# ErickRosete/tacorl

Hardware: AMD Instinct MI355X
Metric: offline grad-steps/sec (batch=256, 84x84 RGB) (higher is better)
Workload: dtype bf16; 1 GPU; tacorl actor-critic training_step, frozen LMP (BASELINE configs[1]); per_gpu_batch=256, global_batch=256, window=16, image=84x84x3, frames=fp32 CHW (reference batch schema), latent_plan=16, n_action_samples=4, phase=Q (epoch>=bc_epochs), action_decoder_loss=every step (reference behaviour), parallelism=dp1, hip_graph=True, losses_finite=True

## Files before the change

### include/tacorl_hip.h

```cpp
#ifndef TACORL_HIP_H
#define TACORL_HIP_H
#include <stddef.h>
#ifdef __cplusplus
extern "C" {
#endif

typedef void* tacorl_stream_t;

#define TACORL_MAXP 16
enum { TACORL_F32 = 0, TACORL_BF16 = 1 };
enum { TACORL_ACT_NONE = 0, TACORL_ACT_RELU = 1, TACORL_ACT_SILU = 2, TACORL_ACT_TANH = 3 };

int tacorl_hip_version(void);
int tacorl_hip_init(int device);
const char* tacorl_hip_last_error(void);
int tacorl_time_mark(unsigned long long* marks, int slot, tacorl_stream_t stream);
int tacorl_time_spin(unsigned long long* marks, int slot, long ticks, tacorl_stream_t stream);

int tacorl_linear_fwd(int nprob, const float* const* x, int ldx, const float* const* w,
                      const float* const* b, float* const* y, float* const* z, const int* M,
                      int K, int N, int act, int compute_dtype, tacorl_stream_t stream);
size_t tacorl_linear_add_fwd_ws_bytes(int nprob, const int* M, int K, int N);
int tacorl_linear_add_fwd(int nprob, const float* const* x, int ldx, const float* const* w,
                          const float* const* b, const float* const* addend, int ld_add, float* const* y,
// ... 161 lines not shown
                               void* ws, size_t ws_bytes, tacorl_stream_t stream);

int tacorl_pack_images(const float* src, long img_pitch, int src_nchw, void* dst, int dst_dtype,
                       int n, int C, int H, int W, tacorl_stream_t stream);
int tacorl_pack_images_batch(int njobs, const float* const* src, const long* img_pitch, void* const* dst,
                             const int* n_img, int dst_dtype, int H, int W, tacorl_stream_t stream);
int tacorl_pack_images_window_batch(int njobs, const float* const* src, const long* img_pitch, void* const* dst,
                                    const int* n_img, void* const* dst_first, void* const* dst_last,
                                    const int* window, int dst_dtype, int H, int W, tacorl_stream_t stream);
int tacorl_pack_images_u8_batch(int njobs, const void* const* src, const long* img_pitch_bytes, void* const* dst,
                                const int* n_img, int dst_dtype, int H, int W, tacorl_stream_t stream);
int tacorl_pack_images_u8_gather_batch(int njobs, const void* const* src, const long* img_pitch_bytes,
                                       const long* const* index, const int* index_stride, void* const* dst,
                                       const int* n_img, int dst_dtype, int H, int W, tacorl_stream_t stream);
int tacorl_gather_frames_u8(const void* frames, long frame_bytes, const long* index, void* dst, long n,
                            tacorl_stream_t stream);
int tacorl_pack_images_u8_aug_batch(int njobs, const void* const* src, const long* img_pitch_bytes,
                                    void* const* dst, const int* const* shift, const float* const* jitter,
                                    const int* n_img, int dst_dtype, int H, int W, int pad,
                                    tacorl_stream_t stream);
int tacorl_pack_images_u8_resize_aug_gather_batch(int njobs, const void* const* src, const long* img_pitch_bytes,
                                                  const long* const* index, const int* index_stride, void* const* dst,
                                                  const int* const* shift, const float* const* jitter, const int* n_img,
                                                  int dst_dtype, int src_H, int src_W, int H, int W, int pad,
                                                  tacorl_stream_t stream);
int tacorl_resize_frames_u8(const void* src, long src_pitch_bytes, void* dst, long dst_pitch_bytes, long n, int src_H,
                            int src_W, int H, int W, tacorl_stream_t stream);
int tacorl_pack_images_u8_aug_gather_batch(int njobs, const void* const* src, const long* img_pitch_bytes,
                                           const long* const* index, const int* index_stride, void* const* dst,
                                           const int* const* shift, const float* const* jitter, const int* n_img,
                                           int dst_dtype, int H, int W, int pad, tacorl_stream_t stream);
int tacorl_stage_transition(const void* disp, int disp_dtype, float* reward, float* done, int B,
                            const float* acts_src, float* acts_dst, long n_acts, tacorl_stream_t stream);
int tacorl_sample_transitions(const long* possible_steps, long n_possible, const long* ep_start, const long* ep_end,
                              int n_episodes, const long* nn_ptr, long n_nn, const long* nn_val, const float* actions,
                              const long* idx, const long* strategy, const long* disp, const double* u_choice,
                              long current_horizon, long n_frames, int B, int A, long* ids, float* action,
                              float* reward, float* done, int* status, tacorl_stream_t stream);
int tacorl_sample_relay(const long* episode_lookup, long n_items, const long* ep_start, const long* ep_end, int n_episodes,
                        const float* actions, long n_frames, const long* idx, const double* u_low, const double* u_high,
                        long max_low_level_window, long max_high_level_window, int B, int A, long* ids, float* action,
                        int* status, tacorl_stream_t stream);
int tacorl_sample_d4rl_windows(const long* episode_lookup, long n_items, const long* ep_start, const long* ep_end,
                               int n_episodes, const float* observations, const float* actions, long n_frames,
                               const long* idx, const long* window, const long* disp, int B, int Tmax, int S, int A,
                               int G, int min_window, float threshold, float* obs, float* act, float* goal,
                               float* reached, float* done, long* window_size, long* ids, int* status,
                               tacorl_stream_t stream);
int tacorl_sample_play_windows(const long* episode_lookup, long n_items, const long* ep_start, const long* ep_end,
                               int n_episodes, const long* nn_ptr, long n_nn, const long* nn_val, const float* actions,
                               long n_frames, long last_end, const long* idx, const long* window, const long* strategy,
                               const long* disp, const long* noise_step, const double* u_choice,
                               const double* u_random_state, int B, int Tmax, int A, int min_window, long* ids, float* act,
                               long* disp_out, long* window_size, int* status, tacorl_stream_t stream);
int tacorl_copy_cols(const float* src, int ld_src, float* dst, int ld_dst, int rows, int cols,
                     int src_row_mod, int accumulate, tacorl_stream_t stream);
int tacorl_copy_cols_batch(int n, const float* const* src, const int* ld_src, float* const* dst,
                           const int* ld_dst, const int* rows, const int* cols,
                           const int* src_row_mod, const int* accumulate, tacorl_stream_t stream);
int tacorl_vec_rows_max_blocks(void);
int tacorl_vec_rows(const float* obs, const float* goal, const float* acts_main, const float* act_pi,
                    const float* act_next, float* const* out, void* const* out_bf16, int B, int T, int S, int G, int A,
                    int n, int lds, int ldq, tacorl_stream_t stream);
int tacorl_reduce_rows_mod(const float* in, int ld_in, float* out, int ld_out, int B, int cols,
                           int reps, tacorl_stream_t stream);
int tacorl_reduce_rows_mod_batch(int n, const float* const* in, int ld_in, float* const* out, int ld_out, int B,
// ... 199 lines not shown
```

### tacorl_amd/_lib.py

```python
import ctypes as C
import os

HERE = os.path.dirname(os.path.abspath(__file__))
LIB_PATH = os.environ.get("TACORL_HIP_LIB") or os.path.join(HERE, "lib", "libtacorl_hip.so")

F32, BF16 = 0, 1
ACT_NONE, ACT_RELU, ACT_SILU, ACT_TANH = 0, 1, 2, 3
MAXP = 16

LOG_SLOTS = [
    "alpha_loss", "alpha", "actor_loss", "bellman_q1_loss", "bellman_q2_loss", "conservative_q1_loss",
    "conservative_q2_loss", "q1_loss", "q2_loss", "alpha_prime", "alpha_prime_loss", "q1_data", "q1_random",
    "q1_policy", "q2_data", "q2_random", "q2_policy", "action_loss",
]

_p, _i, _l, _f, _sz = C.c_void_p, C.c_int, C.c_long, C.c_float, C.c_size_t
_SIGS = {
    "tacorl_hip_version": (_i, []),
    "tacorl_hip_init": (_i, [_i]),
    "tacorl_hip_last_error": (C.c_char_p, []),
    "tacorl_time_mark": (_i, [_p, _i, _p]),
    "tacorl_time_spin": (_i, [_p, _i, _l, _p]),
    "tacorl_linear_fwd": (_i, [_i, _p, _i, _p, _p, _p, _p, _p, _i, _i, _i, _i, _p]),
    "tacorl_linear_add_fwd_ws_bytes": (_sz, [_i, _p, _i, _i]),
# ... 83 lines not shown
    "tacorl_encoder_fused_wpk_bytes": (_l, []),
    "tacorl_encoder_fused_supported": (_i, [_i, _i]),
    "tacorl_encoder_fused_act_format": (_i, [_i, _i]),
    "tacorl_encoder_pack_weights": (_i, [_i, _p, _p, _p]),
    "tacorl_encoder_fwd_fused": (_i, [_i, _p, _p, _p, _p, _p, _p, _i, _i, _p]),
    "tacorl_encoder_fwd_fused_wg": (_i, [_i, _p, _p, _p, _p, _p, _p, _i, _i, _i, _p]),
    "tacorl_encoder_src_entry_bytes": (_l, []),
    "tacorl_encoder_src_supported": (_i, [_p, _l, _l, _l, _i, _i]),
    "tacorl_encoder_src_fill": (_i, [_p, _i, _p, _p, _p, _p, _i, _i, _p]),
    "tacorl_encoder_fwd_fused_src": (_i, [_i, _p, _p, _p, _p, _p, _p, _p, _i, _i, _i, _p]),
    "tacorl_encoder_bwd_fused_ws_bytes": (_sz, [_i, _p, _i, _i]),
    "tacorl_encoder_bwd_fused": (_i, [_i, _p, _p, _p, _p, _p, _p, _i, _i, _i, _p, _sz, _p]),
    "tacorl_encoder_bwd_fused_pack": (_i, [_i, _p, _p, _i, _i, _p, _sz, _p]),
    "tacorl_encoder_bwd_fused_head": (_i, [_i, _p, _p, _p, _p, _i, _i, _i, _p, _sz, _p]),
    "tacorl_encoder_bwd_fused_fc_wgrad": (_i, [_i, _p, _p, _p, _p, _i, _i, _i, _p, _sz, _p]),
    "tacorl_encoder_bwd_fused_conv": (_i, [_i, _p, _p, _p, _p, _p, _i, _i, _i, _i, _p, _sz, _p]),
    "tacorl_encoder_bwd_fused_conv_parts": (_i, [_i, _p, _p, _p, _p, _p, _i, _i, _i, _i, _i, _p, _sz, _p]),
    "tacorl_mlp_param_layout": (_l, [_i, _p, _p, _p]),
    "tacorl_mlp_act_layout": (_l, [_i, _i, _p, _p, _p, _p]),
    "tacorl_mlp_fwd": (_i, [_i, _p, _i, _p, _p, _p, _i, _p, _p, _i, _p]),
    "tacorl_mlp_bwd_ws_bytes": (_sz, [_i, _p, _i, _p]),
    "tacorl_mlp_bwd": (_i, [_i, _p, _i, _p, _p, _p, _i, _p, _p, _i, _p, _i, _p, _p, _i, _i, _p, _sz, _p]),
    "tacorl_pack_images": (_i, [_p, _l, _i, _p, _i, _i, _i, _i, _i, _p]),
    "tacorl_pack_images_batch": (_i, [_i, _p, _p, _p, _p, _i, _i, _i, _p]),
    "tacorl_pack_images_window_batch": (_i, [_i, _p, _p, _p, _p, _p, _p, _p, _i, _i, _i, _p]),
    "tacorl_pack_images_u8_batch": (_i, [_i, _p, _p, _p, _p, _i, _i, _i, _p]),
    "tacorl_pack_images_u8_gather_batch": (_i, [_i, _p, _p, _p, _p, _p, _p, _i, _i, _i, _p]),
    "tacorl_pack_images_u8_aug_gather_batch": (_i, [_i, _p, _p, _p, _p, _p, _p, _p, _p, _i, _i, _i, _i, _p]),
    "tacorl_pack_images_u8_resize_aug_gather_batch": (_i, [_i, _p, _p, _p, _p, _p, _p, _p, _p, _i, _i, _i, _i, _i, _i, _p]),
    "tacorl_gather_frames_u8": (_i, [_p, _l, _p, _p, _l, _p]),
    "tacorl_resize_frames_u8": (_i, [_p, _l, _p, _l, _l, _i, _i, _i, _i, _p]),
    "tacorl_pack_images_u8_aug_batch": (_i, [_i, _p, _p, _p, _p, _p, _p, _i, _i, _i, _i, _p]),
    "tacorl_stage_transition": (_i, [_p, _i, _p, _p, _i, _p, _p, _l, _p]),
    "tacorl_sample_transitions": (_i, [_p, _l, _p, _p, _i, _p, _l, _p, _p, _p, _p, _p, _p, _l, _l, _i, _i, _p, _p, _p, _p, _p, _p]),
    "tacorl_sample_relay": (_i, [_p, _l, _p, _p, _i, _p, _l, _p, _p, _p, _l, _l, _i, _i, _p, _p, _p, _p]),
    "tacorl_sample_d4rl_windows": (_i, [_p, _l, _p, _p, _i, _p, _p, _l, _p, _p, _p, _i, _i, _i, _i, _i, _i, _f, _p, _p, _p, _p, _p, _p,
                                        _p, _p, _p]),
    "tacorl_sample_play_windows": (_i, [_p, _l, _p, _p, _i, _p, _l, _p, _p, _l, _l, _p, _p, _p, _p, _p, _p, _p, _i, _i, _i, _i,
                                        _p, _p, _p, _p, _p, _p]),
    "tacorl_copy_cols": (_i, [_p, _i, _p, _i, _i, _i, _i, _i, _p]),
    "tacorl_copy_cols_batch": (_i, [_i, _p, _p, _p, _p, _p, _p, _p, _p, _p]),
    "tacorl_vec_rows_max_blocks": (_i, []),
    "tacorl_vec_rows": (_i, [_p, _p, _p, _p, _p, _p, _p, _i, _i, _i, _i, _i, _i, _i, _i, _p]),
    "tacorl_reduce_rows_mod": (_i, [_p, _i, _p, _i, _i, _i, _i, _p]),
    "tacorl_reduce_rows_mod_batch": (_i, [_i, _p, _i, _p, _i, _i, _i, _i, _p]),
    "tacorl_uniform_actions": (_i, [_p, _p, _i, _i, _i, _i, _p]),
    "tacorl_tanh_normal_sample": (_i, [_p, _i, _p, _p, _i, _p, _i, _p, _p, _i, _i, _i, _p]),
    "tacorl_tanh_normal_sample_batch": (_i, [_i, _p, _i, _p, _p, _p, _p, _i, _p, _p, _p, _i, _i, _p, _p, _i, _i, _i, _p]),
    "tacorl_alpha_loss": (_i, [_p, _i, _p, _f, _f, _p, _p, _p]),
    "tacorl_alpha_loss_step": (_i, [_p, _i, _p, _f, _p, _p, _p, _p, _f, _p, _p]),
    "tacorl_actor_qmin": (_i, [_p, _p, _p, _i, _p, _p, _p, _f, _p, _p]),
    "tacorl_actor_head_bwd": (_i, [_p, _i, _p, _p, _p, _p, _i, _p, _i, _p, _p, _f, _p, _i, _i, _i, _p, _p]),
    "tacorl_tanh_normal_nll": (_i, [_p, _i, _p, _i, _i, _i, _i, _f, _p, _p, _p]),
    "tacorl_cql_ws_bytes": (_sz, [_i]),
    "tacorl_cql_loss": (_i, [_p] * 13 + [_i, _i, _i, _f, _f, _f, _f, _f, _i, _f, _p, _p, _p, _sz, _p]),
    "tacorl_adam_ws_bytes": (_sz, [_l]),
    "tacorl_adam_step": (_i, [_p, _p, _p, _p, _l, _f, _f, _p, _p, _f, _p, _sz, _p]),
    "tacorl_adam_batch_ws_bytes": (_sz, [_i]),
    "tacorl_adam_step_batch": (_i, [_i, _p, _p, _p, _p, _p, _p, _p, _p, _p, _p, _p, _sz, _p]),
    "tacorl_adam_step_batch_mirror": (_i, [_i, _p, _p, _p, _p, _p, _p, _p, _p, _p, _p, _p, _p, _p, _sz, _p]),
    "tacorl_cem_supported": (_i, [_i, _i, _i, _i, _i, _i]),
    "tacorl_cem_ws_bytes": (_sz, [_i, _i, _i, _i, _i, _i, _i]),
    "tacorl_cem_refine": (_i, [_i, _i, _p, _p, _p, _p, _p, _p, _i, _i, _i, _i, _i, _i, _i, _f, _f, _f, _i, _i, _p, _p, _p, _p, _p,
                               _p, _sz, _p]),
    "tacorl_knn_l2_supported": (_i, [_i, _i]),
    "tacorl_knn_l2_tile": (_i, []),
# ... 94 lines not shown
```

### tacorl_amd/csrc/rl_ops.hip

```cpp
#include <stdio.h>

#include "../../include/tacorl_hip.h"
#include "common.h"

#define LAUNCH_OK() (hipGetLastError() == hipSuccess ? TACORL_OK : TACORL_ELAUNCH)

__device__ __forceinline__ float softplusf(float x) {
  return x > 20.f ? x : log1pf(expf(x));
}
__device__ __forceinline__ float block_sum_256(float v, float* sh) {
  v = wave_sum(v);
  __syncthreads();
  if ((threadIdx.x & 63) == 0) sh[threadIdx.x >> 6] = v;
  __syncthreads();
  return sh[0] + sh[1] + sh[2] + sh[3];
}

template <typename OutT>
__global__ void pack_images_kernel(const float* __restrict__ src, long img_pitch, int src_nchw,
                                   OutT* __restrict__ dst, int n, int C, int HW) {
  const long total = (long)n * HW;
  for (long i = (long)blockIdx.x * blockDim.x + threadIdx.x; i < total; i += (long)gridDim.x * blockDim.x) {
    const long img = i / HW;
    const int px = (int)(i - img * HW);
    const float* s = src + img * img_pitch;
    OutT* d = dst + i * C;
    for (int c = 0; c < C; c++) d[c] = (OutT)(src_nchw ? s[(long)c * HW + px] : s[(long)px * C + c]);
  }
}
extern "C" int tacorl_pack_images(const float* src, long img_pitch, int src_nchw, void* dst, int dst_dtype,
                                  int n, int C, int H, int W, tacorl_stream_t stream) {
  if (n <= 0) return TACORL_OK;
  const long total = (long)n * H * W;
  const int blocks = (int)((total + 255) / 256 > 4096 ? 4096 : (total + 255) / 256);
  if (dst_dtype == TACORL_BF16)
    hipLaunchKernelGGL(pack_images_kernel<__bf16>, dim3(blocks), dim3(256), 0, (hipStream_t)stream, src, img_pitch,
// ... 149 lines not shown
  }
  if (m == 0) return TACORL_OK;
  const int blocks = (int)((mx + 255) / 256 > 8192 ? 8192 : (mx + 255) / 256);
  if (dst_dtype == TACORL_BF16)
    hipLaunchKernelGGL(pack_u8_batch_kernel<__bf16>, dim3(blocks, m), dim3(256), 0, (hipStream_t)stream, t, (int)(bytes / 16));
  else
    hipLaunchKernelGGL(pack_u8_batch_kernel<float>, dim3(blocks, m), dim3(256), 0, (hipStream_t)stream, t, (int)(bytes / 16));
  return LAUNCH_OK();
}

__global__ void stage_transition_kernel(const void* __restrict__ disp, int disp_dtype, float* __restrict__ reward,
                                        float* __restrict__ done, int B, const float* __restrict__ acts_src,
                                        float* __restrict__ acts_dst, long n_acts) {
  const long i = (long)blockIdx.x * blockDim.x + threadIdx.x;
  if (i < B) {
    bool one;
    if (disp_dtype == 0) one = static_cast<const float*>(disp)[i] == 1.0f;
    else if (disp_dtype == 1) one = static_cast<const long long*>(disp)[i] == 1;
    else if (disp_dtype == 2) one = static_cast<const int*>(disp)[i] == 1;
    else one = static_cast<const unsigned char*>(disp)[i] == 1;
    const float r = one ? 1.0f : 0.0f;
    reward[i] = r;
    if (done) done[i] = r;
  }
  for (long k = i; k < n_acts; k += (long)gridDim.x * blockDim.x) acts_dst[k] = acts_src[k];
}
extern "C" int tacorl_stage_transition(const void* disp, int disp_dtype, float* reward, float* done, int B,
                                       const float* acts_src, float* acts_dst, long n_acts, tacorl_stream_t stream) {
  if (!disp || !reward || B < 1 || disp_dtype < 0 || disp_dtype > 3 || (n_acts > 0 && (!acts_src || !acts_dst))) return TACORL_EINVAL;
  const long work = n_acts > B ? n_acts : B;
  const int blocks = (int)((work + 255) / 256 > 1024 ? 1024 : (work + 255) / 256);
  hipLaunchKernelGGL(stage_transition_kernel, dim3(blocks < (B + 255) / 256 ? (B + 255) / 256 : blocks), dim3(256), 0,
                     (hipStream_t)stream, disp, disp_dtype, reward, done, B, acts_src, acts_dst, n_acts);
  return LAUNCH_OK();
}

__global__ void copy_cols_kernel(const float* __restrict__ src, int ld_src, float* __restrict__ dst, int ld_dst,
                                 int rows, int cols, int src_row_mod, int accumulate) {
  const long total = (long)rows * cols;
  for (long i = (long)blockIdx.x * blockDim.x + threadIdx.x; i < total; i += (long)gridDim.x * blockDim.x) {
    const int r = (int)(i / cols), c = (int)(i - (long)r * cols);
    const int rs = src_row_mod > 0 ? r % src_row_mod : r;
    const float v = src[(long)rs * ld_src + c];
    float* d = dst + (long)r * ld_dst + c;
    *d = accumulate ? *d + v : v;
  }
}
extern "C" int tacorl_copy_cols(const float* src, int ld_src, float* dst, int ld_dst, int rows, int cols,
                                int src_row_mod, int accumulate, tacorl_stream_t stream) {
  if (rows <= 0 || cols <= 0) return TACORL_OK;
  const long total = (long)rows * cols;
  const int blocks = (int)((total + 255) / 256 > 2048 ? 2048 : (total + 255) / 256);
  hipLaunchKernelGGL(copy_cols_kernel, dim3(blocks), dim3(256), 0, (hipStream_t)stream, src, ld_src, dst, ld_dst, rows,
                     cols, src_row_mod, accumulate);
  return LAUNCH_OK();
}

#define COPY_MAXB 32
struct CopyTbl {
  const float* src[COPY_MAXB];
  float* dst[COPY_MAXB];
  int ld_src[COPY_MAXB], ld_dst[COPY_MAXB], rows[COPY_MAXB], cols[COPY_MAXB], mod[COPY_MAXB], acc[COPY_MAXB];
};
__global__ void copy_cols_batch_kernel(CopyTbl t) {
  const int d = blockIdx.y, cols = t.cols[d], mod = t.mod[d], acc = t.acc[d];
  const long total = (long)t.rows[d] * cols;
// ... 858 lines not shown
```

### tacorl_amd/encoder_stage.py

```python
import torch

from . import ops
from ._lib import BF16, F32, call

EF_MAXP = 16
EBW_MAXP = 8


def image_flag(img_dtype):
    return BF16 if img_dtype == torch.bfloat16 else F32


def fused_fwd_ok(hw, compute, img_dtype):
    return compute == BF16 and img_dtype == torch.bfloat16 and bool(ops.L.lib().tacorl_encoder_fused_supported(*hw))


def fused_bwd_ok(hw, compute, img_dtype, n_imgs):
    return fused_fwd_ok(hw, compute, img_dtype) and ops.L.lib().tacorl_encoder_bwd_fused_ws_bytes(
        len(n_imgs), ops.int_array(n_imgs), *hw) > 0


def fused_saves(hw, compute, img_dtype, n_imgs):
    return fused_bwd_ok(hw, compute, img_dtype, n_imgs) or (
        fused_fwd_ok(hw, compute, img_dtype) and ops.L.lib().tacorl_encoder_fused_act_format(*hw) == 2)
# ... 38 lines not shown
    for c in cams:
        groups.setdefault((tuple(hw[c]), bool(ok(c))), []).append(c)
    for (_, good), cs in groups.items():
        out += [cs] if good and sum(n_problems(c) for c in cs) <= limit else [[c] for c in cs]
    return out


def problem_src(x):
    return x[7] if len(x) > 7 else None


class SourceTable:

    def __init__(self, device, n):
        self.esz = int(ops.L.lib().tacorl_encoder_src_entry_bytes())
        self.n, self.buf = n, torch.zeros(n * self.esz, dtype=torch.uint8, device=device)

    def entry(self, i):
        return self.buf.data_ptr() + i * self.esz

    @staticmethod
    def ok(base, img_pitch, hw):
        H, W = hw
        return bool(ops.L.lib().tacorl_encoder_src_supported(ops.C.c_void_p(base), img_pitch, H * W, W, H, W))

    def fill(self, sources, hw):
        H, W = hw
        n, Lg = len(sources), ops.C.c_long * len(sources)
        assert 0 < n <= self.n
        call("tacorl_encoder_src_fill", ops.ptr(self.buf), n, ops.ptr_array([b for b, _ in sources]), Lg(*[p for _, p in sources]),
             Lg(*[H * W] * n), Lg(*[W] * n), H, W, ops.stream())


def launch_fused(pr, packs, hw, max_wg=0):
    srcs = [problem_src(x) for x in pr]
    if any(srcs):
        assert not any(s_ and x[5] for s_, x in zip(srcs, pr)), "a problem with a backward reads the packed image"
        call("tacorl_encoder_fwd_fused_src", len(pr), ops.ptr_array([x[0] for x in pr]), ops.ptr_array(srcs),
             ops.ptr_array([packs.buffer(x[1], x[6]) for x in pr]), ops.ptr_array([x[1].enc(x[6]) for x in pr]),
             ops.ptr_array([x[2] for x in pr]), ops.ptr_array([x[3] if x[5] else None for x in pr]),
             ops.int_array([x[4] for x in pr]), *hw, int(max_wg), ops.stream())
        return
    call("tacorl_encoder_fwd_fused_wg", len(pr), ops.ptr_array([x[0] for x in pr]),
         ops.ptr_array([packs.buffer(x[1], x[6]) for x in pr]), ops.ptr_array([x[1].enc(x[6]) for x in pr]),
         ops.ptr_array([x[2] for x in pr]), ops.ptr_array([x[3] if x[5] else None for x in pr]),
         ops.int_array([x[4] for x in pr]), *hw, int(max_wg), ops.stream())


def encode(groups, problems, hw, compute, img_dtype, packs, fused, saves, launch, pack_per_camera=True, per_layer_last=False):
    def per_layer(pr):
        for c in dict.fromkeys(x[6] for x in pr):
            prc = [x for x in pr if x[6] == c]
            call("tacorl_encoder_fwd", len(prc), ops.ptr_array([x[0] for x in prc]), ops.ptr_array([x[1].enc(c) for x in prc]),
                 ops.ptr_array([x[2] for x in prc]), ops.ptr_array([x[3] for x in prc]), ops.int_array([x[4] for x in prc]),
                 *hw[c], image_flag(img_dtype), compute, ops.stream())

    slow = []
    for cs in groups:
        pr = [x for c in cs for x in problems(c)]
        if fused(cs[0]):
            unsaved = lambda x: x[5] and not saves(x[6])
            slow += [x for x in pr if unsaved(x)]
            pr = [x for x in pr if not unsaved(x)]
            pairs = list(dict.fromkeys((x[1], x[6]) for c in cs for x in pr if x[6] == c))
            for part in ([[p for p in pairs if p[1] == c] for c in cs] if pack_per_camera else [pairs]):
                packs.pack_stale(part)
# ... 8 lines not shown
```

### tacorl_amd/modules/tacorl/tacorl.py

```python
import torch

from ... import encoder_stage as stage
from ... import image_ingest as ingest
from ... import ops
from ..._lib import call, ptr
from ...encoder_stage import image_flag
from ..common import register_views
from ..cql.cql_offline_lightning import CQL_Offline
from .latent_plan import LatentPlanShell


class TACORL(LatentPlanShell, CQL_Offline):
    def __init__(self, *args, **kwargs):
        self.action_loss_every_n_steps = kwargs.pop("action_loss_every_n_steps", 1)
        super().__init__(*args, **kwargs)

    def build_networks(self):
        from ..play_lmp.play_lmp_for_rl import PlayLMP, load_play_lmp

        lmp = self.__dict__.pop("_play_lmp", None)
        if lmp is None:
            lmp = load_play_lmp(self.play_lmp_dir, self.lmp_epoch_to_load, self.overwrite_lmp_cfg, device=self.dev,
                                compute_dtype=self.compute, image_dtype=self.img_dtype, unsafe_pickle=self.lmp_unsafe_pickle)
        assert isinstance(lmp, PlayLMP)
# ... 18 lines not shown
            init_views_(q.views)
            n = q.head_off - q.genc_off
            q.param[q.genc_off: q.genc_off + n].copy_(lmp.net.param[lmp.net.genc_off: lmp.net.genc_off + n])
        self.sync_targets()
        self._register()
        self.lmp_net, self.pr, self.ad = lmp.net, lmp.pr, lmp.ad
        enc_views = {k[len("encoder."):]: v for k, v in lmp.net.views.items() if k.startswith("encoder.")}
        register_views(self, "perceptual_encoder.", enc_views, requires_grad=False)
        register_views(self, "plan_recognition.", lmp.pr.blk.views, requires_grad=False)
        if self.ad is not None:
            self._adopt_decoder()
        self._T = None
        from ..inference import attach_rollout_surface

        attach_rollout_surface(self, e.actor, cams, goal_cams, self.action_dim, False, lmp_net=self.lmp_net,
                               lmp_cams=self.action_decoder_modalities, ad=self.ad)

    def _ensure_seq(self, B, T, hw):
        if self._T == (B, T, tuple(sorted(hw.items()))):
            return
        ops.note_alloc()
        dev = self.dev
        self.frames = ingest.LazyImages({c: torch.zeros(B * T, *hw[c], 3, device=dev, dtype=self.img_dtype) for c in self.all_modalities})
        self.f_out = {c: torch.zeros(B * T, 32, device=dev) for c in self.all_modalities}
        self.f_act = {c: torch.zeros(ops.encoder_act_layout(B * T, *hw[c])[1], device=dev) for c in self.all_modalities}
        npr = len(self.plan_recognition_modalities)
        self.pr_in = torch.zeros(B * T, 32 * npr, device=dev)
        e = self.engine
        assert e.action.shape == (B, self.action_dim) and e.action.dtype == torch.float32
        self.plan, self.reward = e.action, e.reward
        self.engine.extra_enc = [dict(cam=c, img=self.frames.raw(c), net=self.lmp_net, out=self.f_out[c],
                                      act=self.f_act[c], n=B * T) for c in self.all_modalities]
        self.src_tbl = {c: stage.SourceTable(dev, 2) for c in sorted(set(self.all_modalities) | set(self.engine.cams))}
        self._folded = None
        self._T = (B, T, tuple(sorted(hw.items())))

    def _stage_small(self, batch, noise, B, T):
        e = self.engine
        disp, acts = batch["disp"], batch["actions"] if self.ad is not None else None
        dd = {torch.float32: 0, torch.int64: 1, torch.int32: 2, torch.uint8: 3, torch.bool: 3}.get(disp.dtype)
        if (dd is not None and disp.is_cuda and disp.is_contiguous() and disp.numel() == B
                and (acts is None or (acts.is_cuda and acts.is_contiguous() and acts.dtype == torch.float32
                                      and acts.shape == self.acts.shape))):
            call("tacorl_stage_transition", ptr(disp), dd, ptr(self.reward), ptr(e.done), B,
                 ptr(acts) if acts is not None else None, ptr(self.acts) if acts is not None else None,
                 acts.numel() if acts is not None else 0, ops.stream())
        else:
            if acts is not None:
                self.acts.copy_(acts)
            self.reward.copy_(disp == 1)
            e.done.copy_(self.reward)
        e.set_noise(noise)

    def _fold_ok(self, f, c, T, batch):
        e, hw = self.engine, f.hw[c]
        if not (f.form == "f32_nchw" and f.aug is None and T >= 2 and e.use_fused and stage.fused_fwd_ok(hw, self.compute, self.img_dtype)):
            return False
        goal = batch["goal"][c] if c in e.cams else None
        if c in e.cams and not (c in e.slot and list(e.slot[c]) == ["obs", "goal", "next"] and goal.is_cuda and goal.is_contiguous()
                                and goal.dtype == torch.float32 and ingest.vector_ok(
                [ingest.PackJob(goal.data_ptr(), 3 * hw[0] * hw[1], 0, 1)], f.form, hw)):
            return False
        v, simg = f.frames[c], 3 * hw[0] * hw[1]
        return stage.SourceTable.ok(v.data_ptr(), simg, hw) and stage.SourceTable.ok(v.data_ptr() + 4 * (T - 1) * simg, T * simg, hw)

    def _stage_frames(self, batch, noise, nchw=True, fold=False):
        from ...data.replay import wait_ready

        wait_ready(batch)
        f = ingest.window_form(batch, nchw)
        B, T, hw, aug = f.B, f.T, f.hw, f.aug
        self.engine.extra_normal = {"eps_pr": (B, self.action_dim)}
        self.engine.ensure_batch(B, {c: hw[c] for c in self.engine.cams})
        self.eps_pr = self.engine.extra_noise["eps_pr"]
        self._ensure_seq(B, T, hw)
        e = self.engine
        if self.ad is not None and (getattr(self, "acts", None) is None or self.acts.shape[:2] != (B, T)):
            ops.note_alloc()
            self.acts = torch.zeros(B, T, 7, device=self.dev)
        if getattr(self, "_stage_stream", None) is None:
            self._stage_stream = torch.cuda.Stream(device=self.dev)
        main = torch.cuda.current_stream()
        side = self._stage_stream if getattr(self, "stage_side", True) else main
        side.wait_stream(main)
        with torch.cuda.stream(side):
            self._stage_small(batch, noise, B, T)
        u8, Job, ip = f.form in ingest.U8_FORMS, ingest.PackJob, None if f.ids is None else f.ids.data_ptr()
        cams_all = sorted(set(self.all_modalities) | set(e.cams))
        for c in cams_all:
            v = f.frames[c]
            assert v.is_cuda and v.is_contiguous() and v.dtype == (torch.uint8 if u8 else torch.float32)
        folded = tuple(c for c in cams_all if fold and self._fold_ok(f, c, T, batch))
        if folded != self._folded:
            ops.note_alloc()
            self._folded = folded
        self.frames.drop()
        e.X3.drop()
        e.fp_src = {c: {"next": self.src_tbl[c].entry(1)} for c in folded if c in e.cams}
        for x in e.extra_enc:
            x["src"] = self.src_tbl[x["cam"]].entry(0) if x["cam"] in folded else None
        for c in cams_all:
            v = f.frames[c]
            src, simg = v.data_ptr(), 3 * f.src_hw[c][0] * f.src_hw[c][1]
            if c in folded:
                self.src_tbl[c].fill([(src, simg), (src + 4 * (T - 1) * simg, T * simg)], hw[c])
                form, shw = f.form, f.src_hw[c]
                later = lambda jobs, c=c, keep=v, form=form, shw=shw: ingest.pack(jobs, form, self.img_dtype, shw, hw[c])
                if c in self.all_modalities:
                    self.frames.defer(c, lambda c=c, later=later, src=src, simg=simg: later([Job(src, simg, self.frames.raw(c).data_ptr(), B * T)]))
                if c in e.cams:
                    x3, slot = e.X3.raw(c).data_ptr(), B * 3 * hw[c][0] * hw[c][1] * e.X3.raw(c).element_size()
                    ingest.pack([Job(src, T * simg, x3, B), Job(batch["goal"][c].data_ptr(), simg, x3 + slot, B)], form, self.img_dtype, shw, hw[c])
                    e.X3.defer(c, lambda later=later, src=src, simg=simg, x3=x3, slot=slot: later([Job(src + 4 * (T - 1) * simg, T * simg, x3 + 2 * slot, B)]))
                continue
            jobs, roles = [], []
            if c in self.all_modalities:
                jobs, roles = [Job(src, simg, self.frames.raw(c).data_ptr(), B * T, ip, 1)], ["window"]
            if c in e.cams:
                x3, slot = e.X3.raw(c).data_ptr(), B * 3 * hw[c][0] * hw[c][1] * e.X3.raw(c).element_size()
                if ip is not None:
                    jobs += [Job(src, simg, x3, B, ip, T), Job(src, simg, x3 + slot, B, ip + 8 * B * T, 1),
                             Job(src, simg, x3 + 2 * slot, B, ip + 8 * (T - 1), T)]
                else:
                    g = batch["goal"][c]
                    assert g.is_cuda and g.is_contiguous() and g.dtype == v.dtype
                    jobs += [Job(src, T * simg, x3, B), Job(g.data_ptr(), simg, x3 + slot, B),
                             Job(src + v.element_size() * (T - 1) * simg, T * simg, x3 + 2 * slot, B)]
                roles += ["obs", "goal", "next"]
            if aug is not None:
                jobs = [j._replace(**ingest.window_tables(aug, c, r, T)) for j, r in zip(jobs, roles)]
            if len(jobs) == 4 and T >= 2 and ingest.vector_ok(jobs, f.form, hw[c]):
                ingest.pack_window(jobs, T, self.img_dtype, hw[c])
            else:
                ingest.pack(jobs, f.form, self.img_dtype, f.src_hw[c], hw[c], aug["pad"][c] if aug is not None else None)
        main.wait_stream(side)
        return B, T, hw

    def _ad_due(self):
        k = self.action_loss_every_n_steps
        return self.ad is not None and (self.finetune_action_decoder or k <= 1 or (self._step_count + 1) % k == 0)

    def _device_front(self, B, T, hw, optimize, with_ad=True):
        e = self.engine
        ops.mark("front:start")
        if getattr(self, "_pr_stream", None) is None:
            self._pr_stream, self._side_stream = torch.cuda.Stream(device=self.dev), torch.cuda.Stream(device=self.dev)
        main = torch.cuda.current_stream()
        mods = self.plan_recognition_modalities
        emb, ld = (self.f_out[mods[0]], 32) if len(mods) == 1 else (self.pr_in, self.pr_in.shape[1])
        ad_prep, ad_prepared = None, False
        if (with_ad and optimize and self.finetune_action_decoder and getattr(self, "ad_early_prepare", True)
                and self.ad._bwd_fast(B, self.compute)):
            self._side_stream.wait_stream(main)
            with torch.cuda.stream(self._side_stream):
                self.ad.refresh_mirrors(B, T - 1)
                ad_prepared = self.ad.prepare_backward(B, T - 1, self.compute)
                ad_prep = torch.cuda.Event()
                ad_prep.record(self._side_stream)
        split = with_ad and (T >= 24 or (optimize and self.finetune_action_decoder))
        forked = []

        def fork_branches():
            forked.append(self._fork_pr_ad(B, T, main, mods, emb, ld, with_ad, optimize, ad_prep, ad_prepared))

        if not (split and e.encode_split(fork_branches)):
            e._encode_all()
        ops.mark("front:encoded")
        if not forked:
            fork_branches()
        ready, ad_on_side = forked[0]
        e.action_ready = ready
        e.phase_a(encoded=True, optimize=optimize)
        if ad_prep is not None:
            main.wait_stream(self._side_stream)
        segmented = self._segmented() or not self._use_graph
        if with_ad and not ad_on_side:
            if segmented:
# ... 28 lines not shown
            ready = torch.cuda.Event()
            ready.record(self._pr_stream)
            if with_ad and not ad_on_side:
                if ad_prep is not None:
                    self._pr_stream.wait_event(ad_prep)
                self.ad.loss_step(self, self.acts, self.plan, B, T, True, defer_update=self._defer_ad_update(),
                                  mirrors_current=ad_prep is not None, prepared=ad_prepared)
        if ad_on_side:
            self._side_stream.wait_event(ready)
            with torch.cuda.stream(self._side_stream):
                ops.mark("ad:start")
                self.ad.loss_step(self, self.acts, self.plan, B, T, False, frozen=not self.finetune_action_decoder,
                                  rows_current=rows_current)
                ops.mark("ad:end")
            self._ad_join = self._side_stream
        return ready, ad_on_side

    def get_pr_latent_plan(self, batch, noise=None, nchw=True):
        B, T, hw = self._stage_frames(batch, noise, nchw)
        xd = image_flag(self.img_dtype)
        for c in self.all_modalities:
            H, W = hw[c]
            call("tacorl_encoder_fwd", 1, ops.ptr_array([self.frames[c]]), ops.ptr_array([self.lmp_net.enc(c)]),
                 ops.ptr_array([self.f_out[c]]), ops.ptr_array([self.f_act[c]]), ops.int_array([B * T]), H, W, xd,
                 self.compute, ops.stream())
        for j, c in enumerate(self.plan_recognition_modalities):
            ops.copy_cols(self.f_out[c], 0, 32, self.pr_in, 32 * j, self.pr_in.shape[1], B * T, 32)
        head = self.pr.forward(self.pr_in, self.pr_in.shape[1], B, T, self.compute, inference=True)
        call("tacorl_pr_sample", ptr(head), ptr(self.eps_pr), ptr(self.plan), None, None, B, self.action_dim,
             float(self.pr.min_std), ops.stream())
        return self.plan

    def _step(self, batch, noise, optimize, log_type, nchw=True):
        B, T, hw = self._stage_frames(batch, noise, nchw, fold=getattr(self, "fp32_ingest", True))
        with_ad = self._ad_due()
        key = ("tacorl", B, T, tuple(sorted(hw.items())), self.current_epoch < self.bc_epochs, optimize, with_ad)
        e, bc = self.engine, self.current_epoch < self.bc_epochs
        ad_update = with_ad and optimize and self.finetune_action_decoder and self._defer_ad_update()

        def tail():
            e.phase_c(optimize)
            self._join_ad()
            if ad_update:
                self.ad.update(self)
            ops.mark("step:end")

        segmented = self._segmented()
        ad_ft = optimize and self.finetune_action_decoder
        ad_side = with_ad and segmented and self._use_graph
        side = None
        if ad_side and ad_ft:
            side = (0, lambda: self.ad.loss_step(self, self.acts, self.plan, B, T, True, defer_update=True), 1)
        elif ad_side:
            side = (0, lambda: self.ad.loss_step(self, self.acts, self.plan, B, T, False, frozen=not self.finetune_action_decoder))
        def allreduce_grads():
            if ad_update:
                self._join_ad()
            e.allreduce_grads()

        self._run_segments(key, [lambda: self._device_front(B, T, hw, optimize, with_ad and not ad_side),
                                 lambda: e.phase_b(bc, optimize), tail],
                           [e.allreduce_alpha, allreduce_grads], side=side)
        self._publish_logs(log_type, extra=("action_loss",) if with_ad else ())
```

Before: 1314 grad-steps/s.

## Merge step-front staging into one table-driven kernel launched inside the graph

Replaces the separate per-step front kernels (transition staging, reward/done/action copy, goal and current-frame packing, per-camera source-table fills) with a single device table filled once per step and one step_front kernel launched at the start of the device front. The aim is to cut launch count and the gaps between small kernels and side-stream syncs before the encoder runs. In exchange it adds a fill kernel plus host-side table assembly. It also moves staging onto the main stream, which gives up the earlier overlap on the side stream. It only applies when the configuration is non-segmented and all cameras share one folded resolution.

```diff
diff --git a/include/tacorl_hip.h b/include/tacorl_hip.h
--- a/include/tacorl_hip.h
+++ b/include/tacorl_hip.h
@@ -217,6 +217,22 @@
                                            int dst_dtype, int H, int W, int pad, tacorl_stream_t stream);
 int tacorl_stage_transition(const void* disp, int disp_dtype, float* reward, float* done, int B,
                             const float* acts_src, float* acts_dst, long n_acts, tacorl_stream_t stream);
+#define TACORL_SF_MAXCAM 4
+#define TACORL_SF_MAXJOBS 8
+#define TACORL_SF_NOFFSETS 15
+long tacorl_step_front_table_bytes(void);
+int tacorl_step_front_offsets(long* offsets);
+int tacorl_step_front_supported(int nsrc, const float* const* src_base, const long* src_pitch, int njobs,
+                                const float* const* pack_src, const long* pack_pitch, void* const* pack_dst,
+                                const int* pack_n, const void* disp, int disp_dtype, const float* reward, int B,
+                                const float* acts_src, const float* acts_dst, long n_acts, int H, int W);
+int tacorl_step_front_assemble(void* host_table, int nsrc, const float* const* src_base, const long* src_pitch, int njobs,
+                               const float* const* pack_src, const long* pack_pitch, void* const* pack_dst,
+                               const int* pack_n, const void* disp, int disp_dtype, float* reward, float* done, int B,
+                               const float* acts_src, float* acts_dst, long n_acts, int H, int W);
+int tacorl_step_front_fill(void* table, const void* host_table, tacorl_stream_t stream);
+int tacorl_step_front(const void* table, int njobs, int max_images, int B, long n_acts, int H, int W,
+                      tacorl_stream_t stream);
 int tacorl_sample_transitions(const long* possible_steps, long n_possible, const long* ep_start, const long* ep_end,
                               int n_episodes, const long* nn_ptr, long n_nn, const long* nn_val, const float* actions,
                               const long* idx, const long* strategy, const long* disp, const double* u_choice,
diff --git a/scratch/front_launches.py b/scratch/front_launches.py
--- /dev/null
+++ b/scratch/front_launches.py
@@ -0,0 +1,25 @@
+import csv, glob, sys, collections
+f = glob.glob(sys.argv[1] + "/**/*kernel_trace.csv", recursive=True)[0]
+rows = sorted(csv.DictReader(open(f)), key=lambda r: int(r["Start_Timestamp"]))
+name = lambda r: r["Kernel_Name"].replace("(anonymous namespace)::", "").replace("void ", "")
+enc = [i for i, r in enumerate(rows) if name(r).startswith("encoder_fused_kernel")]
+FRONT = ("pack_nchw3", "stage_transition", "ef_src_fill", "step_front", "distribution", "normal", "uniform")
+for k in (150, 180):
+    a = enc[k]
+    i = a - 1
+    while i > 0 and any(s in name(rows[i]) for s in FRONT):
+        i -= 1
+    t0 = int(rows[i]["End_Timestamp"])
+    print(f"-- step {k}: us since the previous replay's last kernel ended (start, duration, queue, kernel)")
+    for r in rows[i - 1:a + 2]:
+        d = (int(r["End_Timestamp"]) - int(r["Start_Timestamp"])) / 1e3
+        print(f"{(int(r['Start_Timestamp']) - t0) / 1e3:9.1f} us  {d:7.1f}  q{r.get('Queue_Id', '?')}  {name(r)[:100]}")
+tot, cnt = collections.Counter(), collections.Counter()
+for r in rows:
+    n = name(r)
+    if any(s in n for s in FRONT) or n.startswith("encoder_fused_kernel"):
+        tot[n[:80]] += (int(r["End_Timestamp"]) - int(r["Start_Timestamp"])) / 1e3
+        cnt[n[:80]] += 1
+print("-- mean us per dispatch (dispatches)")
+for n in tot:
+    print(f"{tot[n] / cnt[n]:8.1f}  ({cnt[n]})  {n}")
diff --git a/scratch/front_marks.py b/scratch/front_marks.py
--- /dev/null
+++ b/scratch/front_marks.py
@@ -0,0 +1,31 @@
+import os, sys, json
+sys.path.insert(0, os.path.join(os.path.dirname(os.path.abspath(__file__)), ".."))
+import torch, bench
+from tacorl_amd import _lib, ops
+dev = torch.device("cuda:0"); _lib.call("tacorl_hip_init", 0)
+res = {}
+for traced in (False, True):
+    reader = ops.trace_marks(dev) if traced else None
+    mod = bench.build_module(dev, "bf16", 16, 1)
+    batch = bench.synth_batch(256, 16, 84, 84, dev, 1)
+    mod.enable_graph(); mod.log_every_n_steps = 50
+    def run(n):
+        for i in range(n): mod.training_step(batch, i)
+    run(20); torch.cuda.synchronize()
+    per, spans, fronts = [], [], []
+    for burst in range(6):
+        e0, e1 = torch.cuda.Event(enable_timing=True), torch.cuda.Event(enable_timing=True)
+        e0.record(); run(200); e1.record(); torch.cuda.synchronize()
+        ms = e0.elapsed_time(e1) / 200
+        per.append(ms)
+        if traced:
+            m = dict(reader())
+            span = m["step:end"] - m["front:start"]
+            spans.append(span); fronts.append(ms * 1000 - span)
+    key = "traced" if traced else "untraced"
+    res[key + "_ms_per_step"] = [round(x, 4) for x in per]
+    if traced:
+        res["span_us"] = [round(x, 1) for x in spans]
+        res["front_us"] = [round(x, 1) for x in fronts]
+        res["last_marks"] = [(n, round(t, 1)) for n, t in reader()]
+print("FRONT " + json.dumps(res), flush=True)
diff --git a/tacorl_amd/_lib.py b/tacorl_amd/_lib.py
--- a/tacorl_amd/_lib.py
+++ b/tacorl_amd/_lib.py
@@ -139,6 +139,12 @@
     "tacorl_resize_frames_u8": (_i, [_p, _l, _p, _l, _l, _i, _i, _i, _i, _p]),
     "tacorl_pack_images_u8_aug_batch": (_i, [_i, _p, _p, _p, _p, _p, _p, _i, _i, _i, _i, _p]),
     "tacorl_stage_transition": (_i, [_p, _i, _p, _p, _i, _p, _p, _l, _p]),
+    "tacorl_step_front_table_bytes": (_l, []),
+    "tacorl_step_front_offsets": (_i, [_p]),
+    "tacorl_step_front_supported": (_i, [_i, _p, _p, _i, _p, _p, _p, _p, _p, _i, _p, _i, _p, _p, _l, _i, _i]),
+    "tacorl_step_front_assemble": (_i, [_p, _i, _p, _p, _i, _p, _p, _p, _p, _p, _i, _p, _p, _i, _p, _p, _l, _i, _i]),
+    "tacorl_step_front_fill": (_i, [_p, _p, _p]),
+    "tacorl_step_front": (_i, [_p, _i, _i, _i, _l, _i, _i, _p]),
     "tacorl_sample_transitions": (_i, [_p, _l, _p, _p, _i, _p, _l, _p, _p, _p, _p, _p, _p, _l, _l, _i, _i, _p, _p, _p, _p, _p, _p]),
     "tacorl_sample_relay": (_i, [_p, _l, _p, _p, _i, _p, _l, _p, _p, _p, _l, _l, _i, _i, _p, _p, _p, _p]),
     "tacorl_sample_d4rl_windows": (_i, [_p, _l, _p, _p, _i, _p, _p, _l, _p, _p, _p, _i, _i, _i, _i, _i, _i, _f, _p, _p, _p, _p, _p, _p,
diff --git a/tacorl_amd/csrc/rl_ops.hip b/tacorl_amd/csrc/rl_ops.hip
--- a/tacorl_amd/csrc/rl_ops.hip
+++ b/tacorl_amd/csrc/rl_ops.hip
@@ -1,7 +1,11 @@
+#include <stddef.h>
 #include <stdio.h>
+#include <string.h>
 
 #include "../../include/tacorl_hip.h"
 #include "common.h"
+#include "encoder_fused.h"
+#include "step_front_table.h"
 
 #define LAUNCH_OK() (hipGetLastError() == hipSuccess ? TACORL_OK : TACORL_ELAUNCH)
 
@@ -217,6 +221,114 @@
   const int blocks = (int)((work + 255) / 256 > 1024 ? 1024 : (work + 255) / 256);
   hipLaunchKernelGGL(stage_transition_kernel, dim3(blocks < (B + 255) / 256 ? (B + 255) / 256 : blocks), dim3(256), 0,
                      (hipStream_t)stream, disp, disp_dtype, reward, done, B, acts_src, acts_dst, n_acts);
+  return LAUNCH_OK();
+}
+
+static_assert(sizeof(SFSrc) == sizeof(EFSrc) && offsetof(SFSrc, base) == offsetof(EFSrc, base) &&
+                  offsetof(SFSrc, img_pitch) == offsetof(EFSrc, img_pitch) && offsetof(SFSrc, plane_pitch) == offsetof(EFSrc, plane_pitch) &&
+                  offsetof(SFSrc, row_pitch) == offsetof(EFSrc, row_pitch),
+              "the front table's source entries are the fused encoder's");
+__global__ void step_front_fill_kernel(SFTable* __restrict__ tbl, SFTable f) {
+  const long* s = reinterpret_cast<const long*>(&f);
+  long* d = reinterpret_cast<long*>(tbl);
+  for (int i = threadIdx.x; i < (int)(sizeof(SFTable) / 8); i += blockDim.x) d[i] = s[i];
+}
+__global__ void step_front_kernel(const SFTable* __restrict__ t) {
+  const int j = blockIdx.y;
+  if (j < t->njobs) {
+    const int HW = t->HW, q4 = HW / 4;
+    const long total = (long)t->pack_n[j] * q4, pitch = t->pack_pitch[j];
+    const float* __restrict__ src = t->pack_src[j];
+    __bf16* __restrict__ dst = reinterpret_cast<__bf16*>(t->pack_dst[j]);
+    for (long q = (long)blockIdx.x * blockDim.x + threadIdx.x; q < total; q += (long)gridDim.x * blockDim.x) {
+      const long img = q / q4;
+      const int p = (int)(q - img * q4) * 4;
+      const float* s = src + img * pitch + p;
+      const f32x4 r = *reinterpret_cast<const f32x4*>(s), g = *reinterpret_cast<const f32x4*>(s + HW),
+                  b = *reinterpret_cast<const f32x4*>(s + 2 * HW);
+      const float v[12] = {r[0], g[0], b[0], r[1], g[1], b[1], r[2], g[2], b[2], r[3], g[3], b[3]};
+      __bf16* d = dst + (img * HW + p) * 3;
+#pragma unroll
+      for (int k = 0; k < 3; k++)
+        *reinterpret_cast<bf16x4*>(d + 4 * k) = bf16x4{(__bf16)v[4 * k], (__bf16)v[4 * k + 1], (__bf16)v[4 * k + 2], (__bf16)v[4 * k + 3]};
+    }
+    return;
+  }
+  if (j != (int)gridDim.y - 1) return;
+  const long i = (long)blockIdx.x * blockDim.x + threadIdx.x;
+  const int B = t->B, disp_dtype = t->disp_dtype;
+  const void* __restrict__ disp = t->disp;
+  if (i < B) {
+    bool one;
+    if (disp_dtype == 0) one = static_cast<const float*>(disp)[i] == 1.0f;
+    else if (disp_dtype == 1) one = static_cast<const long long*>(disp)[i] == 1;
+    else if (disp_dtype == 2) one = static_cast<const int*>(disp)[i] == 1;
+    else one = static_cast<const unsigned char*>(disp)[i] == 1;
+    const float r = one ? 1.0f : 0.0f;
+    t->reward[i] = r;
+    if (t->done) t->done[i] = r;
+  }
+  const long n_acts = t->n_acts;
+  const float* __restrict__ acts_src = t->acts_src;
+  float* __restrict__ acts_dst = t->acts_dst;
+  for (long k = i; k < n_acts; k += (long)gridDim.x * blockDim.x) acts_dst[k] = acts_src[k];
+}
+extern "C" long tacorl_step_front_table_bytes(void) { return (long)sizeof(SFTable); }
+extern "C" int tacorl_step_front_offsets(long* out) {
+  if (!out) return TACORL_EINVAL;
+  const long o[TACORL_SF_NOFFSETS] = {
+      (long)offsetof(SFTable, src),      (long)offsetof(SFTable, pack_src),   (long)offsetof(SFTable, pack_dst),
+      (long)offsetof(SFTable, pack_pitch), (long)offsetof(SFTable, pack_n),   (long)offsetof(SFTable, disp),
+      (long)offsetof(SFTable, reward),   (long)offsetof(SFTable, done),       (long)offsetof(SFTable, acts_src),
+      (long)offsetof(SFTable, acts_dst), (long)offsetof(SFTable, n_acts),     (long)offsetof(SFTable, disp_dtype),
+      (long)offsetof(SFTable, B),        (long)offsetof(SFTable, njobs),      (long)offsetof(SFTable, HW)};
+  for (int i = 0; i < TACORL_SF_NOFFSETS; i++) out[i] = o[i];
+  return TACORL_OK;
+}
+extern "C" int tacorl_step_front_supported(int nsrc, const float* const* src_base, const long* src_pitch, int njobs,
+                                           const float* const* pack_src, const long* pack_pitch, void* const* pack_dst,
+                                           const int* pack_n, const void* disp, int disp_dtype, const float* reward, int B,
+                                           const float* acts_src, const float* acts_dst, long n_acts, int H, int W) {
+  if (!sf_supported(nsrc, src_base, src_pitch, njobs, pack_src, pack_pitch, pack_dst, pack_n, disp, disp_dtype, reward, B, acts_src,
+                    acts_dst, n_acts, H, W))
+    return 0;
+  for (int i = 0; i < nsrc; i++)
+    if (!tacorl_encoder_src_supported(src_base[i], src_pitch[i], (long)H * W, W, H, W)) return 0;
+  return 1;
+}
+extern "C" int tacorl_step_front_assemble(void* host_table, int nsrc, const float* const* src_base, const long* src_pitch,
+                                          int njobs, const float* const* pack_src, const long* pack_pitch,
+                                          void* const* pack_dst, const int* pack_n, const void* disp, int disp_dtype,
+                                          float* reward, float* done, int B, const float* acts_src, float* acts_dst,
+                                          long n_acts, int H, int W) {
+  if (!host_table || !tacorl_step_front_supported(nsrc, src_base, src_pitch, njobs, pack_src, pack_pitch, pack_dst, pack_n, disp,
+                                                  disp_dtype, reward, B, acts_src, acts_dst, n_acts, H, W))
+    return TACORL_EINVAL;
+  sf_assemble(static_cast<SFTable*>(host_table), nsrc, src_base, src_pitch, njobs, pack_src, pack_pitch, pack_dst, pack_n, disp,
+              disp_dtype, reward, done, B, acts_src, acts_dst, n_acts, H, W);
+  return TACORL_OK;
+}
+extern "C" int tacorl_step_front_fill(void* table, const void* host_table, tacorl_stream_t stream) {
+  if (!table || !host_table || ((uintptr_t)table & 7)) return TACORL_EINVAL;
+  SFTable f;
+  memcpy(&f, host_table, sizeof(SFTable));
+  if (!sf_table_sane(f)) return TACORL_EINVAL;
+  hipLaunchKernelGGL(step_front_fill_kernel, dim3(1), dim3(64), 0, (hipStream_t)stream, static_cast<SFTable*>(table), f);
+  return LAUNCH_OK();
+}
+extern "C" int tacorl_step_front(const void* table, int njobs, int max_images, int B, long n_acts, int H, int W,
+                                 tacorl_stream_t stream) {
+  if (!table || njobs < 0 || njobs > TACORL_SF_MAXJOBS || (njobs > 0 && max_images < 1) || B < 1 || n_acts < 0 || H < 1 || W < 1 ||
+      ((long)H * W) % 4)
+    return TACORL_EINVAL;
+  const long pack = njobs > 0 ? ((long)max_images * (H * W / 4) + 255) / 256 : 0;
+  const long work = n_acts > B ? n_acts : B;
+  long blocks = pack > 8192 ? 8192 : pack;
+  const long small = (work + 255) / 256 > 1024 ? 1024 : (work + 255) / 256;
+  if (njobs == 0) blocks = small;
+  if (blocks < ((long)B + 255) / 256) blocks = ((long)B + 255) / 256;
+  hipLaunchKernelGGL(step_front_kernel, dim3((unsigned)blocks, njobs + 1), dim3(256), 0, (hipStream_t)stream,
+                     static_cast<const SFTable*>(table));
   return LAUNCH_OK();
 }
 
diff --git a/tacorl_amd/csrc/step_front_table.h b/tacorl_amd/csrc/step_front_table.h
--- /dev/null
+++ b/tacorl_amd/csrc/step_front_table.h
@@ -0,0 +1,62 @@
+#pragma once
+#include <stdint.h>
+#include <string.h>
+
+#include "../../include/tacorl_hip.h"
+
+struct SFSrc {
+  const float* base;
+  long img_pitch, plane_pitch, row_pitch;
+};
+struct SFTable {
+  SFSrc src[2 * TACORL_SF_MAXCAM];
+  const float* pack_src[TACORL_SF_MAXJOBS];
+  void* pack_dst[TACORL_SF_MAXJOBS];
+  long pack_pitch[TACORL_SF_MAXJOBS];
+  int pack_n[TACORL_SF_MAXJOBS];
+  const void* disp;
+  float* reward;
+  float* done;
+  const float* acts_src;
+  float* acts_dst;
+  long n_acts;
+  int disp_dtype, B;
+  int njobs, HW;
+};
+
+inline bool sf_supported(int nsrc, const float* const* src_base, const long* src_pitch, int njobs, const float* const* pack_src,
+                         const long* pack_pitch, void* const* pack_dst, const int* pack_n, const void* disp, int disp_dtype,
+                         const float* reward, int B, const float* acts_src, const float* acts_dst, long n_acts, int H, int W) {
+  if (nsrc < 0 || nsrc > 2 * TACORL_SF_MAXCAM || njobs < 0 || njobs > TACORL_SF_MAXJOBS || H < 1 || W < 1 || ((long)H * W) % 4)
+    return false;
+  if ((nsrc > 0 && (!src_base || !src_pitch)) || (njobs > 0 && (!pack_src || !pack_pitch || !pack_dst || !pack_n))) return false;
+  for (int i = 0; i < nsrc; i++)
+    if (!src_base[i] || ((uintptr_t)src_base[i] & 15) || src_pitch[i] % 4 || src_pitch[i] < 0) return false;
+  for (int j = 0; j < njobs; j++)
+    if (!pack_src[j] || !pack_dst[j] || ((uintptr_t)pack_src[j] & 15) || ((uintptr_t)pack_dst[j] & 15) || pack_pitch[j] % 4 ||
+        pack_pitch[j] < 0 || pack_n[j] < 1)
+      return false;
+  if (!disp || !reward || B < 1 || disp_dtype < 0 || disp_dtype > 3) return false;
+  return n_acts == 0 || (n_acts > 0 && acts_src && acts_dst);
+}
+
+inline void sf_assemble(SFTable* t, int nsrc, const float* const* src_base, const long* src_pitch, int njobs,
+                        const float* const* pack_src, const long* pack_pitch, void* const* pack_dst, const int* pack_n,
+                        const void* disp, int disp_dtype, float* reward, float* done, int B, const float* acts_src,
+                        float* acts_dst, long n_acts, int H, int W) {
+  memset(t, 0, sizeof(SFTable));
+  for (int i = 0; i < nsrc; i++) {
+    t->src[i].base = src_base[i]; t->src[i].img_pitch = src_pitch[i];
+    t->src[i].plane_pitch = (long)H * W; t->src[i].row_pitch = W;
+  }
+  for (int j = 0; j < njobs; j++) {
+    t->pack_src[j] = pack_src[j]; t->pack_dst[j] = pack_dst[j]; t->pack_pitch[j] = pack_pitch[j]; t->pack_n[j] = pack_n[j];
+  }
+  t->disp = disp; t->reward = reward; t->done = done;
+  t->acts_src = n_acts > 0 ? acts_src : nullptr; t->acts_dst = n_acts > 0 ? acts_dst : nullptr; t->n_acts = n_acts;
+  t->disp_dtype = disp_dtype; t->B = B; t->njobs = njobs; t->HW = H * W;
+}
+
+inline bool sf_table_sane(const SFTable& f) {
+  return f.njobs >= 0 && f.njobs <= TACORL_SF_MAXJOBS && f.B >= 1 && f.HW >= 4 && f.HW % 4 == 0 && f.disp_dtype >= 0 && f.disp_dtype <= 3;
+}
diff --git a/tacorl_amd/encoder_stage.py b/tacorl_amd/encoder_stage.py
--- a/tacorl_amd/encoder_stage.py
+++ b/tacorl_amd/encoder_stage.py
@@ -94,6 +94,48 @@
              Lg(*[H * W] * n), Lg(*[W] * n), H, W, ops.stream())
 
 
+class FrontTable:
+
+    def __init__(self, device):
+        L = ops.L.lib()
+        self.nbytes, self.esz = int(L.tacorl_step_front_table_bytes()), int(L.tacorl_encoder_src_entry_bytes())
+        offs = (ops.C.c_long * 15)()
+        call("tacorl_step_front_offsets", offs)
+        self.src_off = int(offs[0])
+        self.buf = torch.zeros(self.nbytes, dtype=torch.uint8, device=device)
+        self.host = ops.C.create_string_buffer(self.nbytes)
+        self.plan = self.bytes = self.shadow = self.grid = None
+
+    def entry(self, cam, which):
+        return self.buf.data_ptr() + self.src_off + (2 * cam + which) * self.esz
+
+    def invalidate(self):
+        self.shadow = None
+
+    def accept(self, plan):
+        if plan != self.plan:
+            sources, jobs, disp, disp_dtype, reward, done, B, acts_src, acts_dst, n_acts, hw = plan
+            Ls, Lj = ops.C.c_long * len(sources), ops.C.c_long * len(jobs)
+            if ops.L.lib().tacorl_step_front_assemble(
+                    self.host, len(sources), ops.ptr_array([b for b, _ in sources]), Ls(*[p for _, p in sources]), len(jobs),
+                    ops.ptr_array([j.src for j in jobs]), Lj(*[j.pitch for j in jobs]), ops.ptr_array([j.dst for j in jobs]),
+                    ops.int_array([j.n for j in jobs]), disp, disp_dtype, reward, done, B, acts_src, acts_dst, n_acts, *hw) != 0:
+                return False
+            self.plan, self.bytes = plan, self.host.raw
+            self.grid = (len(jobs), max([j.n for j in jobs], default=0), B, n_acts, *hw)
+        return True
+
+    def commit(self):
+        if self.bytes == self.shadow:
+            return False
+        call("tacorl_step_front_fill", ops.ptr(self.buf), self.bytes, ops.stream())
+        self.shadow = self.bytes
+        return True
+
+    def launch(self):
+        call("tacorl_step_front", ops.ptr(self.buf), *self.grid, ops.stream())
+
+
 def launch_fused(pr, packs, hw, max_wg=0):
     srcs = [problem_src(x) for x in pr]
     if any(srcs):
diff --git a/tacorl_amd/modules/tacorl/tacorl.py b/tacorl_amd/modules/tacorl/tacorl.py
--- a/tacorl_amd/modules/tacorl/tacorl.py
+++ b/tacorl_amd/modules/tacorl/tacorl.py
@@ -74,16 +74,25 @@
         self.engine.extra_enc = [dict(cam=c, img=self.frames.raw(c), net=self.lmp_net, out=self.f_out[c],
                                       act=self.f_act[c], n=B * T) for c in self.all_modalities]
         self.src_tbl = {c: stage.SourceTable(dev, 2) for c in sorted(set(self.all_modalities) | set(self.engine.cams))}
-        self._folded = None
+        self.front_tbl = stage.FrontTable(dev)
+        self._folded = self._front = None
         self._T = (B, T, tuple(sorted(hw.items())))
 
-    def _stage_small(self, batch, noise, B, T):
-        e = self.engine
+    def _small_sources(self, batch, B):
         disp, acts = batch["disp"], batch["actions"] if self.ad is not None else None
         dd = {torch.float32: 0, torch.int64: 1, torch.int32: 2, torch.uint8: 3, torch.bool: 3}.get(disp.dtype)
         if (dd is not None and disp.is_cuda and disp.is_contiguous() and disp.numel() == B
                 and (acts is None or (acts.is_cuda and acts.is_contiguous() and acts.dtype == torch.float32
                                       and acts.shape == self.acts.shape))):
+            return disp, dd, acts
+        return None
+
+    def _stage_small(self, batch, noise, B, T):
+        e = self.engine
+        disp, acts = batch["disp"], batch["actions"] if self.ad is not None else None
+        small = self._small_sources(batch, B)
+        if small is not None:
+            dd = small[1]
             call("tacorl_stage_transition", ptr(disp), dd, ptr(self.reward), ptr(e.done), B,
                  ptr(acts) if acts is not None else None, ptr(self.acts) if acts is not None else None,
                  acts.numel() if acts is not None else 0, ops.stream())
@@ -106,7 +115,25 @@
         v, simg = f.frames[c], 3 * hw[0] * hw[1]
         return stage.SourceTable.ok(v.data_ptr(), simg, hw) and stage.SourceTable.ok(v.data_ptr() + 4 * (T - 1) * simg, T * simg, hw)
 
-    def _stage_frames(self, batch, noise, nchw=True, fold=False):
+    def _front_plan(self, f, batch, B, T, cams_all, folded):
+        e, Job = self.engine, ingest.PackJob
+        small = self._small_sources(batch, B)
+        if not folded or folded != tuple(cams_all) or small is None or len({tuple(f.hw[c]) for c in cams_all}) != 1:
+            return None
+        disp, dd, acts = small
+        sources, jobs = [], []
+        for c in cams_all:
+            src, simg = f.frames[c].data_ptr(), 3 * f.hw[c][0] * f.hw[c][1]
+            sources += [(src, simg), (src + 4 * (T - 1) * simg, T * simg)]
+            if c in e.cams:
+                x3, slot = e.X3.raw(c).data_ptr(), B * simg * e.X3.raw(c).element_size()
+                jobs += [Job(src, T * simg, x3, B), Job(batch["goal"][c].data_ptr(), simg, x3 + slot, B)]
+        plan = (tuple(sources), tuple(jobs), disp.data_ptr(), dd, self.reward.data_ptr(), e.done.data_ptr(), B,
+                acts.data_ptr() if acts is not None else None, self.acts.data_ptr() if acts is not None else None,
+                acts.numel() if acts is not None else 0, tuple(f.hw[cams_all[0]]))
+        return plan if self.front_tbl.accept(plan) else None
+
+    def _stage_frames(self, batch, noise, nchw=True, fold=False, front=False):
         from ...data.replay import wait_ready
 
         wait_ready(batch)
@@ -123,36 +150,50 @@
         if getattr(self, "_stage_stream", None) is None:
             self._stage_stream = torch.cuda.Stream(device=self.dev)
         main = torch.cuda.current_stream()
-        side = self._stage_stream if getattr(self, "stage_side", True) else main
-        side.wait_stream(main)
-        with torch.cuda.stream(side):
-            self._stage_small(batch, noise, B, T)
         u8, Job, ip = f.form in ingest.U8_FORMS, ingest.PackJob, None if f.ids is None else f.ids.data_ptr()
         cams_all = sorted(set(self.all_modalities) | set(e.cams))
         for c in cams_all:
             v = f.frames[c]
             assert v.is_cuda and v.is_contiguous() and v.dtype == (torch.uint8 if u8 else torch.float32)
         folded = tuple(c for c in cams_all if fold and self._fold_ok(f, c, T, batch))
-        if folded != self._folded:
+        plan = self._front_plan(f, batch, B, T, cams_all, folded) if front else None
+        if folded != self._folded or (plan is not None) != self._front:
             ops.note_alloc()
-            self._folded = folded
+            self.front_tbl.invalidate()
+            self._folded, self._front = folded, plan is not None
+        side = self._stage_stream if getattr(self, "stage_side", True) else main
+        if plan is not None:
+            side = main
+            self.front_tbl.commit()
+            self._front_keep = (batch["goal"], batch["disp"], batch.get("actions"))
+        if side is not main:
+            side.wait_stream(main)
+        with torch.cuda.stream(side):
+            if plan is not None:
+                e.set_noise(noise)
+            else:
+                self._stage_small(batch, noise, B, T)
         self.frames.drop()
         e.X3.drop()
-        e.fp_src = {c: {"next": self.src_tbl[c].entry(1)} for c in folded if c in e.cams}
+        tbl_i = {c: i for i, c in enumerate(cams_all)}
+        entry = (lambda c, k: self.front_tbl.entry(tbl_i[c], k)) if plan is not None else (lambda c, k: self.src_tbl[c].entry(k))
+        e.fp_src = {c: {"next": entry(c, 1)} for c in folded if c in e.cams}
         for x in e.extra_enc:
-            x["src"] = self.src_tbl[x["cam"]].entry(0) if x["cam"] in folded else None
+            x["src"] = entry(x["cam"], 0) if x["cam"] in folded else None
         for c in cams_all:
             v = f.frames[c]
             src, simg = v.data_ptr(), 3 * f.src_hw[c][0] * f.src_hw[c][1]
             if c in folded:
-                self.src_tbl[c].fill([(src, simg), (src + 4 * (T - 1) * simg, T * simg)], hw[c])
+                if plan is None:
+                    self.src_tbl[c].fill([(src, simg), (src + 4 * (T - 1) * simg, T * simg)], hw[c])
                 form, shw = f.form, f.src_hw[c]
                 later = lambda jobs, c=c, keep=v, form=form, shw=shw: ingest.pack(jobs, form, self.img_dtype, shw, hw[c])
                 if c in self.all_modalities:
                     self.frames.defer(c, lambda c=c, later=later, src=src, simg=simg: later([Job(src, simg, self.frames.raw(c).data_ptr(), B * T)]))
                 if c in e.cams:
                     x3, slot = e.X3.raw(c).data_ptr(), B * 3 * hw[c][0] * hw[c][1] * e.X3.raw(c).element_size()
-                    ingest.pack([Job(src, T * simg, x3, B), Job(batch["goal"][c].data_ptr(), simg, x3 + slot, B)], form, self.img_dtype, shw, hw[c])
+                    if plan is None:
+                        ingest.pack([Job(src, T * simg, x3, B), Job(batch["goal"][c].data_ptr(), simg, x3 + slot, B)], form, self.img_dtype, shw, hw[c])
                     e.X3.defer(c, lambda later=later, src=src, simg=simg, x3=x3, slot=slot: later([Job(src + 4 * (T - 1) * simg, T * simg, x3 + 2 * slot, B)]))
                 continue
             jobs, roles = [], []
@@ -175,7 +216,8 @@
                 ingest.pack_window(jobs, T, self.img_dtype, hw[c])
             else:
                 ingest.pack(jobs, f.form, self.img_dtype, f.src_hw[c], hw[c], aug["pad"][c] if aug is not None else None)
-        main.wait_stream(side)
+        if side is not main:
+            main.wait_stream(side)
         return B, T, hw
 
     def _ad_due(self):
@@ -185,6 +227,8 @@
     def _device_front(self, B, T, hw, optimize, with_ad=True):
         e = self.engine
         ops.mark("front:start")
+        if self._front:
+            self.front_tbl.launch()
         if getattr(self, "_pr_stream", None) is None:
             self._pr_stream, self._side_stream = torch.cuda.Stream(device=self.dev), torch.cuda.Stream(device=self.dev)
         main = torch.cuda.current_stream()
@@ -279,7 +323,7 @@
         return self.plan
 
     def _step(self, batch, noise, optimize, log_type, nchw=True):
-        B, T, hw = self._stage_frames(batch, noise, nchw, fold=getattr(self, "fp32_ingest", True))
+        B, T, hw = self._stage_frames(batch, noise, nchw, fold=getattr(self, "fp32_ingest", True), front=not self._segmented())
         with_ad = self._ad_due()
         key = ("tacorl", B, T, tuple(sorted(hw.items())), self.current_epoch < self.bc_epochs, optimize, with_ad)
         e, bc = self.engine, self.current_epoch < self.bc_epochs
```

Result: faster. 1353 grad-steps/s, median of 6 (+3.0%).
